# ywq/psnerf

Measured on AMD Instinct MI355X. Metric: ray-samples/sec (train step) on BEAR stage2, higher is better.
Workload: dtype f32

## Files before the change

### include/psnerf_hip.h

```cpp
#ifndef PSNERF_HIP_H
#define PSNERF_HIP_H

#include <stdint.h>

#ifdef __cplusplus
extern "C" {
#endif

#define PSN_OK 0
#define PSN_E_ARG (-1)
#define PSN_E_LAUNCH (-2)
#define PSN_E_UNSUPPORTED (-3)

const char* psn_last_error(void);
int psn_version(void);

int psn_composite_fwd(const float* alpha, const float* rgb, int64_t n_rays, int n_samples, int white_bg,
                      float* weights, float* rgb_out, float* acc_out, void* stream);
int psn_composite_bwd(const float* alpha, const float* rgb, const float* d_rgb_out, const float* d_acc_out,
                      int64_t n_rays, int n_samples, int white_bg, float* d_alpha, float* d_rgb, void* stream);

int psn_pe_encode(const float* x, int64_t n, int n_freqs, float scale, float* out, int out_stride, void* stream);
int psn_app_input(const float* p, const float* v, const float* normal, int64_t n, int n_freqs, float* out, void* stream);

// ... 222 lines not shown
int psn_stage1_rays(const float* pix, const float* camera_mat, int k_ld, const float* world_mat, float radius2, int64_t n,
                    float* cam, float* rays, float* far, void* stream);
int psn_surface_points(const float* d_pred, const int* flags, const float* cam, const float* rays, int64_t n, float* d_i,
                       float* dists, unsigned char* obj_mask, float* points, void* stream);
int psn_stage1_targets(const float* pix, int64_t n, int h, int w, const float* img, const float* mask, const float* mask_valid,
                       const float* normal, const float* norm_mask, const float* world_mat, int use_angle, float cos_thresh,
                       float* rgb_gt, float* mask_gt, unsigned char* mask_valid_out, float* normal_gt,
                       unsigned char* norm_mask_out, void* stream);
#define PSN_COPY2D_MAX 24
typedef struct {
    const float* src; int64_t ld_src;
    float* dst; int64_t ld_dst;
    int rows, cols;
} PsnCopy2dItem;
int psn_copy2d_group(int n_items, const PsnCopy2dItem* items, void* stream);
#define PSN_COPY_BYTES_MAX 24
typedef struct { const void* src; void* dst; int64_t n_bytes; int aligned; } PsnCopyBytesItem;
int psn_copy_bytes_group(int n_items, const PsnCopyBytesItem* items, void* stream);
int psn_mask_count(const unsigned char* mask_a, const unsigned char* mask_b, int64_t n, float* out, void* stream);
int psn_surface_index(const unsigned char* mask, int64_t n, int64_t cap, int64_t* idx, float* count, void* stream);
int psn_inverse_index(const int64_t* idx, int64_t ns, int64_t n_pix, int* inv, const float* count, void* stream);
typedef struct {
    const void* images; int image_type; const float* lut;
    const unsigned char* object_mask; const unsigned char* surface_mask;
    const float* points; const float* normal; const float* visibility; const float* vis_plus; const float* light_direction;
    int64_t hw; int width;
    const int64_t* lidx; int n_lights;
    const int64_t* pix; int64_t pix0; int64_t n;
    const int64_t* vidx; int n_vis;
    float* rgb; unsigned char* object_mask_out; unsigned char* surface_mask_out; float* uv; float* points_out; float* normal_out;
// ... 170 lines not shown
```

### psnerf_amd/csrc/small.hip

```cpp
#include "common.h"

namespace psn {

__device__ __forceinline__ void normalize3(const float x0, const float x1, const float x2, float eps, float& y0, float& y1, float& y2) {
    const float nrm = sqrtf(x0 * x0 + x1 * x1 + x2 * x2);
    const float d = nrm < eps ? eps : nrm;
    y0 = x0 / d; y1 = x1 / d; y2 = x2 / d;
}
__device__ __forceinline__ void normalize3_bwd(const float x0, const float x1, const float x2, const float g0, const float g1,
                                               const float g2, float eps, float& d0, float& d1, float& d2) {
    const float nrm = sqrtf(x0 * x0 + x1 * x1 + x2 * x2);
    const float d = nrm < eps ? eps : nrm;
    d0 = g0 / d; d1 = g1 / d; d2 = g2 / d;
    if (nrm >= eps && nrm > 0.0f) {
        const float s = -((g0 * x0 / d) / d + (g1 * x1 / d) / d + (g2 * x2 / d) / d);
        d0 += x0 / nrm * s; d1 += x1 / nrm * s; d2 += x2 / nrm * s;
    }
}

__global__ __launch_bounds__(256) void normalize_rows_fwd_kernel(const float* __restrict__ x, int64_t n, float eps, float* __restrict__ y) {
    const int64_t i = (int64_t)blockIdx.x * 256 + threadIdx.x;
    if (i >= n) return;
    float y0, y1, y2;
    normalize3(x[3 * i], x[3 * i + 1], x[3 * i + 2], eps, y0, y1, y2);
// ... 224 lines not shown
    Copy2dArgs a;
    a.n = n_items;
    a.start[0] = 0;
    for (int i = 0; i < n_items; ++i) {
        const PsnCopy2dItem& it = items[i];
        PSN_CHECK_ARG(it.src && it.dst && it.rows >= 1 && it.cols >= 1 && it.ld_src >= it.cols && it.ld_dst >= it.cols, "copy2d_group: item %d", i);
        a.it[i] = it;
        a.start[i + 1] = a.start[i] + ((int64_t)it.rows * it.cols + 255) / 256;
    }
    hipLaunchKernelGGL(copy2d_group_kernel, dim3((unsigned)a.start[n_items]), dim3(256), 0, (hipStream_t)stream, a);
    PSN_CHECK_LAUNCH("copy2d_group");
    return PSN_OK;
}

namespace psn {
struct CopyBytesArgs { PsnCopyBytesItem it[PSN_COPY_BYTES_MAX]; int64_t start[PSN_COPY_BYTES_MAX + 1]; int n; };
__global__ __launch_bounds__(256) void copy_bytes_group_kernel(CopyBytesArgs a) {
    int i = 0;
    while (i + 1 < a.n && (int64_t)blockIdx.x >= a.start[i + 1]) ++i;
    const PsnCopyBytesItem it = a.it[i];
    const int64_t b = (int64_t)blockIdx.x - a.start[i];
    const int64_t off = (b * 256 + threadIdx.x) * 16;
    if (off >= it.n_bytes) return;
    const char* s = reinterpret_cast<const char*>(it.src) + off;
    char* d = reinterpret_cast<char*>(it.dst) + off;
    if (it.aligned && off + 16 <= it.n_bytes) {
        *reinterpret_cast<uint4*>(d) = *reinterpret_cast<const uint4*>(s);
    } else {
        const int m = (int)(it.n_bytes - off < 16 ? it.n_bytes - off : 16);
        for (int k = 0; k < m; ++k) d[k] = s[k];
// ... 240 lines not shown
```

### psnerf_amd/fused.py

```python
import math

import torch

from . import hip


class PackCache(object):

    def __init__(self):
        self.epoch = 0
        self._slots = {}

    def key(self, params):
        return (self.epoch,) + tuple((int(p._version), p.data_ptr()) for p in params)

    def invalidate(self):
        self.epoch += 1

    def get(self, slot, params, build, extra=()):
        key = (self.key(params), extra)
        hit = self._slots.get(slot)
        if hit is None or hit[0] != key:
            with torch.no_grad():
                pack = build(hit[1] if hit is not None else None)
# ... 5 lines not shown

    def __init__(self, *args, **kwargs):
        super().__init__(*args, **kwargs)
        self.packs = PackCache()

    def invalidate_packs(self):
        self.packs.invalidate()

    def _apply(self, fn, *a, **k):
        self.packs.invalidate()
        return super()._apply(fn, *a, **k)

    def _load_from_state_dict(self, *a, **k):
        self.packs.invalidate()
        return super()._load_from_state_dict(*a, **k)


def interleave(weights, biases):
    return [t for pair in zip(weights, biases) for t in pair]


class PackedMLP(object):
    def __init__(self, desc, w, b, init_wa=None, init_wb=None, init_bias=None):
        self.desc, self.w, self.b = desc, w, b
        self.init_wa, self.init_wb, self.init_bias = init_wa, init_wb, init_bias
        self.macs_per_row = None

    def on_points(self, points, pe_octaves, pe_scale, out=None, n_rows_dev=None, out_rows=None):
        return hip.mlp_infer_pe(self.desc, self.w, self.b, points, pe_octaves, pe_scale, out=out, macs_per_row=self.macs_per_row,
                                n_rows_dev=n_rows_dev, out_rows=out_rows)
# ... 48 lines not shown

class Transposed(object):

    def __init__(self, w):
        self.w = w.detach()


def _src(w):
    if isinstance(w, Transposed):
        m = w.w
        return m, True, m.shape[1], m.shape[0]
    m = w.detach()
    return m, False, m.shape[0], m.shape[1]


def pack_layers(layers, in_kt_a, in_kt_b, n_out, out_act, device, has_final=True, width=256, reuse=None, x3=False):
    assert width in (64, 128, 256) and (not x3 or width == 256)
    hid = width // 32
    kin = in_kt_a + in_kt_b
    desc = hip.PsnMlpDesc()
    desc.n_layers = len(layers)
    desc.n_out, desc.out_act, desc.in_kt_a, desc.in_kt_b = n_out, out_act, in_kt_a, in_kt_b
    desc.w_format = hip.W_BF16X2 if x3 else hip.W_F32
    assert len(layers) <= hip.MAX_LAYERS
    plan, biases = [], []
    init_wa, init_wb, init_bias = [], [], []
    direct_init_off = None
    off = b_off = 0
    for li, L in enumerate(layers):
        last = has_final and li == len(layers) - 1
        n_mt = (2 if n_out > 32 else 1) if last else hid
# ... 39 lines not shown
        b_buf = _zeros(n_bias, device)
    elif old_b is not None and old_b.numel() == n_bias and old_b.device == w_buf.device and getattr(reuse, 'b_zero', None) == is_zero:
        b_buf, o = old_b, 0
        for bv, z in zip(biases, is_zero):
            if not z:
                side.append((bv, b_buf[o:o + bv.shape[0]]))
            o += bv.shape[0]
    else:
        b_buf = torch.cat(biases).contiguous()
    group = []
    for w, n_mt, k_tiles, o in plan:
        m, tr, r, c = _src(w)
        assert r <= n_mt * 32 and c <= k_tiles * 32, 'pack_layers: block %dx%d does not fit %dx%d' % (r, c, n_mt * 32, k_tiles * 32)
        group.append((m if m.dtype == torch.float32 else m.float(), tr, n_mt, k_tiles, w_buf[o:o + n_mt * k_tiles * 1024],
                      hip.W_BF16X2 if (x3 and n_mt >= 2) else hip.W_F32))
    hip.mlp_pack_layers(group)
    desc.init_stride = width * len(init_wa) if direct_init_off is None else width
    if init_wa:
        def stack(blocks, cols, old):
            shape = (len(blocks) * width, cols)
            buf = old if (old is not None and tuple(old.shape) == shape and old.device == w_buf.device) else torch.zeros(shape, device=device)
            for i, blk in enumerate(blocks):
                assert blk.shape[0] <= width and blk.shape[1] <= cols
                side.append((blk if blk.dtype == torch.float32 else blk.float(), buf[i * width:i * width + blk.shape[0], :blk.shape[1]]))
            return buf
        n_ib = sum(v.shape[0] for v in init_bias)
        old_ib = getattr(reuse, 'init_bias', None)
        if old_ib is not None and old_ib.numel() == n_ib and old_ib.device == w_buf.device:
            ib, o = old_ib, 0
            for v in init_bias:
                side.append((v, ib[o:o + v.shape[0]]))
# ... 4 lines not shown
                       stack(init_wb, in_kt_b * 32, getattr(reuse, 'init_wb', None)) if init_wb else None, ib)
    else:
        pk = PackedMLP(desc, w_buf, b_buf)
    pk.b_zero = is_zero
    if side:
        side = [(a_.detach().contiguous() if a_.dim() == 1 else a_.detach(), d_) for a_, d_ in side]
        if all(a_.is_cuda for a_, _ in side):
            hip.copy2d_group(side)
        else:
            for a_, d_ in side:
                d_.copy_(a_)
    pk.macs_per_row = sum(_src(w)[2] * _src(w)[3] for w, _, _, _ in plan)
    return pk


def pack_relu_mlp(weights, biases, din_a, din_b, skip_at, out_act=hip.OUT_NONE, precompute=True, width=256, reuse=None, x3=False):
    ka = (din_a + 31) // 32
    kb = (din_b + 31) // 32 if din_b > 0 else 0

    def split_in(w):
        if kb == 0:
            return w[:, :din_a]
        wa = _pad_cols(w[:, :din_a], ka * 32)
        return torch.cat([wa, _pad_cols(w[:, din_a:din_a + din_b], kb * 32)], dim=1)

    def in_block(W):
        if precompute:
            return dict(init_a=W[:, :din_a], init_b=W[:, din_a:din_a + din_b] if kb else None)
        return dict(w_in=split_in(W))

    layers = []
    n = len(weights)
    for li in range(n):
        W, b = weights[li].detach(), biases[li].detach()
        act = hip.ACT_RELU if li < n - 1 else hip.ACT_NONE
        if li == 0:
            layers.append(dict(w_act=None, bias=b, act=act, **in_block(W)))
        elif li - 1 == skip_at:
            layers.append(dict(w_act=W[:, :width], bias=b, act=act, **in_block(W[:, width:])))
        else:
            layers.append(dict(w_act=W, bias=b, act=act))
    assert all(L['bias'].shape[0] == width for L in layers[:-1]), 'fused path: every hidden layer must have the given width'
    return pack_layers(layers, ka, kb, weights[-1].shape[0], out_act, weights[0].device, width=width, reuse=reuse, x3=x3)


class PackedBf16(object):

    def __init__(self, desc, w, final_bias):
        self.desc, self.w, self.final_bias = desc, w, final_bias

    def __call__(self, tab_a, n_rows, a_div=1, a_mod=None, tab_b=None, b_div=1, b_mod=1, out=None):
        if a_mod is None:
            a_mod = tab_a.shape[0]
        return hip.mlp_infer_bf16(self.desc, self.w, self.final_bias, tab_a, a_div, a_mod, tab_b, b_div, b_mod, n_rows, out=out)


def pack_relu_mlp_bf16(weights, biases, din_a, din_b, skip_at, out_act=hip.OUT_NONE):
    n = len(weights)
# ... 126 lines not shown
                W, b = -W, -b
        if li == 0:
            layers.append(dict(w_in=W, w_act=None, bias=b, act=act))
        elif li in skips:
            d_x = W.shape[1] - d_pe
            layers.append(dict(w_in=W[:, d_x:] * inv, w_act=W[:, :d_x] * inv, bias=b, act=act))
        else:
            layers.append(dict(w_in=None, w_act=W, bias=b, act=act))
    return pack_layers(layers, ka, 0, 1, out_act, weights[0].device, x3=x3)


def pack_geo_logit(weights, biases, skips, d_pe):
    return pack_geo_occupancy(weights, biases, skips, d_pe, out_act=hip.OUT_NONE, negate=True)


def pack_relu_bwd(weights, skip_at, width=256, bits=False, x3=False):
    n = len(weights)
    dev = weights[0].device
    zeros = _zeros(width, dev)
    act = hip.ACT_RELU_BITS if bits else hip.ACT_RELU_MASK
    layers = [dict(init_a=DIRECT_INIT, init_b=None, w_act=None, bias=zeros, act=act)]
    for l in range(n - 2, 0, -1):
        layers.append(dict(w_act=Transposed(weights[l][:, :width]), bias=zeros, act=act))
    return pack_layers(layers, 1, 0, 0, hip.OUT_NONE, dev, has_final=False, width=width, x3=x3 and width == 256)


def _t(w):
    return Transposed(w)


def pack_geo_chains(weights, biases, skips, d_pe, x3=False):
    n = len(weights)
    assert len(skips) == 1 and weights[1].shape[1] == 256 and weights[n - 1].shape[0] == 257
    sk = skips[0]
    dev = weights[0].device
    W = [w.detach() for w in weights]
    b = [x.detach() for x in biases]
    zeros = _zeros(256, dev)
    ka = (d_pe + 31) // 32
# ... 160 lines not shown
```

### psnerf_amd/hip.py

```python
import ctypes
import os

import torch

from . import cabi

_HERE = os.path.dirname(os.path.abspath(__file__))
LIB_PATH = os.path.join(_HERE, 'libpsnerf_hip.so')

if not os.path.exists(LIB_PATH):
    raise ImportError(
        'psnerf_amd: %s is missing. Build it with `python -m psnerf_amd.build` (hipcc, gfx950). '
        'There is no fallback path.' % LIB_PATH)
_lib = ctypes.CDLL(LIB_PATH)

HEADER_PATH = os.path.join(_HERE, '..', 'include', 'psnerf_hip.h')
if not os.path.exists(HEADER_PATH):
    raise ImportError('psnerf_amd: %s is missing: the binding is derived from it. There is no fallback path.' % HEADER_PATH)

_constants, _structs, SIGNATURES = cabi.parse(HEADER_PATH)
globals().update({_k[len('PSN_'):]: _v for _k, _v in _constants.items()})
globals().update(_structs)
MAX_LAYERS = MLP_MAX_LAYERS
for _name, (_res, _args) in SIGNATURES.items():
# ... 411 lines not shown
    _check(_lib.psn_row_adam(len(items), ctypes.addressof(arr), idx.data_ptr(), idx.numel(), _stream()), 'row_adam')


def normalize_rows_fwd(x, eps=1e-12):
    assert x.dim() == 2 and x.shape[1] == 3 and x.is_contiguous()
    y = torch.empty_like(x)
    _check(_lib.psn_normalize_rows_fwd(_tptr(x, 'x'), x.shape[0], float(eps), y.data_ptr(), _stream()), 'normalize_rows_fwd')
    return y


def normalize_rows_bwd(x, g, eps=1e-12):
    assert x.shape == g.shape and x.shape[1] == 3 and x.is_contiguous() and g.is_contiguous()
    dx = torch.empty_like(x)
    _check(_lib.psn_normalize_rows_bwd(_tptr(x, 'x'), _tptr(g, 'g'), x.shape[0], float(eps), dx.data_ptr(), _stream()), 'normalize_rows_bwd')
    return dx


def light_rows_fwd(dir_table, int_table, idx, eps=1e-12):
    L = idx.shape[0]
    assert dir_table.dim() == 2 and dir_table.shape[1] == 3 and dir_table.is_contiguous() and idx.dtype == torch.int64 and idx.is_contiguous()
    d = torch.empty(L, 3, device=dir_table.device, dtype=torch.float32)
    it = None
    if int_table is not None:
        assert int_table.shape == (dir_table.shape[0], 1) and int_table.is_contiguous()
        it = torch.empty(L, 1, device=dir_table.device, dtype=torch.float32)
    _check(_lib.psn_light_rows_fwd(_tptr(dir_table, 'dir_table'), _tptr(int_table, 'int_table', allow_none=True), _tptr(idx, 'idx', torch.int64), L, float(eps),
                                   d.data_ptr(), None if it is None else it.data_ptr(), _stream()), 'light_rows_fwd')
    return d, it


# ... 1131 lines not shown
```

### psnerf_amd/ops.py

```python
import collections

import torch

from . import fused, hip


HITS = collections.Counter()


def _hit(name):
    HITS[name] += 1


import os as _os0
STRICT = _os0.environ.get('PSN_STRICT', '0') == '1'
FALLBACKS = collections.Counter()


def fallback(name, tensor=None, why=''):
    if tensor is not None and not getattr(tensor, 'is_cuda', False):
        return
    FALLBACKS[name] += 1
    if STRICT:
        raise RuntimeError('psnerf_amd.ops.STRICT: %s left the fused engines on a device tensor%s' % (name, (' (' + why + ')') if why else ''))
# ... 208 lines not shown
class SplitRows(torch.autograd.Function):

    @staticmethod
    def forward(ctx, t, k):
        ctx.k, ctx.shape = k, t.shape
        return t[:k], t[k:]

    @staticmethod
    def backward(ctx, ga, gb):
        k, shape = ctx.k, ctx.shape
        if ga is None:
            ga = gb.new_zeros((k,) + tuple(shape[1:]))
        if gb is None:
            gb = ga.new_zeros((shape[0] - k,) + tuple(shape[1:]))
        return torch.cat([ga, gb], dim=0), None


class ScatterRows(torch.autograd.Function):

    @staticmethod
    def forward(ctx, idx, inv, specs, *rows):
        _hit('ScatterRows')
        ctx.set_materialize_grads(False)
        ctx.specs, ctx.n_pix, ctx.ns = specs, inv.numel(), idx.numel()
        ctx.save_for_backward(idx, inv)
        return tuple(hip.scatter_rows(list(specs), [r.detach() for r in rows], inv, inv.numel(), idx.numel()))

    @staticmethod
    def backward(ctx, *grads):
        idx, inv = ctx.saved_tensors
# ... 285 lines not shown
def mf_shade(light_dir, view, normal, albedo, rough, light_int, vis, f0):
    return MFShade.apply(light_dir, view, normal, albedo, rough, light_int, vis, f0)


RELU_SIGN_BITS = True


def _sign_bits(rows, n, device):
    return [torch.empty(rows, 4, device=device, dtype=torch.int64) for _ in range(n)]


class VisibilityPair(torch.autograd.Function):

    @staticmethod
    def launch(pe_x, pe_l, n_shade, in_cols, skip_at, params, need_grad, packed=None, live_count=None):
        Ws, bs = params[0::2], params[1::2]
        Ns, LV = pe_x.shape[0], pe_l.shape[0]
        V = LV - n_shade
        n = len(Ws)
        din_half = in_cols.numel() // 2
        with torch.no_grad():
            if packed is None:
                packed = fused.pack_relu_mlp(list(Ws), list(bs), din_half, din_half, skip_at)
            save = [torch.empty(V * Ns, 256, device=pe_x.device) for _ in range(n - 1)] if (need_grad and V > 0) else None
            bits = _sign_bits(V * Ns, n - 1, pe_x.device) if (save is not None and RELU_SIGN_BITS) else None
            out = packed(pe_x, LV * Ns, a_div=1, a_mod=Ns, tab_b=pe_l, b_div=Ns, b_mod=LV, save=save, save_row0=n_shade * Ns,
                         live=None if (live_count is None or Ns % 64 != 0) else (live_count, Ns),
                         save_bits=bits)
        return out, (save, bits) if save is not None else None

    @staticmethod
    def forward(ctx, pe_x, pe_l, n_shade, in_cols, skip_at, pre, *params):
        _hit('VisibilityPair')
        Ns, LV = pe_x.shape[0], pe_l.shape[0]
        V = LV - n_shade
        n = len(params) // 2
        need = any(ctx.needs_input_grad[6:])
        out, dumps = pre if pre is not None else VisibilityPair.launch(pe_x, pe_l, n_shade, in_cols, skip_at, params, need)
        save, bits = dumps if (need and dumps is not None) else (None, None)
        if save is not None:
            ctx.save_for_backward(pe_x, pe_l[n_shade:], in_cols, *save, *params)
        ctx.bits = bits
        ctx.n, ctx.skip_at, ctx.V, ctx.saved = n, skip_at, V, save is not None
        ctx.contiguous_cols = bool(getattr(in_cols, '_psn_contiguous_pair', False))
        vis, vis_t = out[:n_shade * Ns], out[n_shade * Ns:]
        ctx.mark_non_differentiable(vis)
        return vis, vis_t

    @staticmethod
    def backward(ctx, _g_vis, g):
        n, V = ctx.n, ctx.V
        if not ctx.saved or g is None:
            return (None,) * (6 + 2 * n)
        sv = ctx.saved_tensors
        pe_x, pe_lv, in_cols = sv[0], sv[1], sv[2]
        H = sv[3:3 + n - 1]
        Ws = sv[3 + n - 1::2]
        Ns = pe_x.shape[0]
        Q = V * Ns
        half = in_cols.numel() // 2
        cols_a, cols_b = in_cols[:half], in_cols[half:] - pe_x.shape[1]
        contiguous_cols = ctx.contiguous_cols
        grads = [None] * (2 * n)
        g = g.contiguous()

        bits = ctx.bits
        chain = fused.pack_relu_bwd(list(Ws), ctx.skip_at, bits=bits is not None, x3=CHAIN_X3)
        DZ = [torch.empty(Q, 256, device=g.device) for _ in range(n - 1)]
        chain(None, Q, a_div=1, a_mod=Q, rank_init=(g.reshape(Q, 1), Ws[n - 1].reshape(1, -1).contiguous()),
              mask=[(bits if bits is not None else H)[n - 2 - j] for j in range(n - 1)], save=DZ, save_row0=0)
        grads[2 * (n - 1)] = hip.colsum(H[n - 2], row_weight=g)
        grads[2 * (n - 1) + 1] = _rowsum_small(g)
        items = []
        where = []
        xl = {}
        for li in range(n - 2, -1, -1):
            dz = DZ[n - 2 - li]
            if li > 0:
                items.append(dict(A=dz, B=H[li - 1], colsum=True))
                where.append((li, 'w'))
            if li == 0 or li - 1 == ctx.skip_at:
                if V <= 16:
# ... 182 lines not shown
        d_feat = torch.empty(Q, 256, device=dev)
        d_normal = chains['bwd'](None, Q, a_div=1, a_mod=Q, rank_init=(g, Ws[n - 1].contiguous()),
                                 mask=[H[n - 2 - j] for j in range(n - 1)] + [None, None], save=DZ + [d_feat])
        dz0 = DZ[n - 2]
        items = [dict(A=dz0, B=x[:, :d_x], colsum=True), dict(A=dz0, B=feat)]
        items += [dict(A=DZ[n - 2 - l], B=H[l - 1], colsum=True) for l in range(1, n - 1)]
        res = hip.gemm_tn_grouped(items)
        grads = [torch.cat([res[0][0], res[1][0]], dim=1), res[0][1]]
        for l in range(1, n - 1):
            grads += [res[l + 1][0], res[l + 1][1]]
        grads += [hip.colsum(H[n - 2], row_weight=g), _rowsum_small(g)]
        return (None, d_normal, d_feat, None, None) + tuple(grads)


class FusedReluNet(torch.autograd.Function):

    @staticmethod
    def pack(Ws, bs, din, skip_at, final_sigmoid, width):
        with torch.no_grad():
            return fused.pack_relu_mlp(list(Ws), list(bs), din, 0, skip_at,
                                       out_act=hip.OUT_SIGMOID if final_sigmoid else hip.OUT_NONE, precompute=False, width=width)

    @staticmethod
    def forward(ctx, pe, din, skip_at, final_sigmoid, width, packed, *params):
        _hit('FusedReluNet')
        Ws, bs = params[0::2], params[1::2]
        n = len(Ws)
        Q = pe.shape[0]
        if packed is None:
            packed = FusedReluNet.pack(Ws, bs, din, skip_at, final_sigmoid, width)
        need = any(ctx.needs_input_grad[6:])
        H = [torch.empty(Q, width, device=pe.device) for _ in range(n - 1)] if need else None
        bits = _sign_bits(Q, n - 1, pe.device) if (need and RELU_SIGN_BITS) else None
        out = packed(pe, Q, save=H, save_bits=bits)
        if need:
            ctx.save_for_backward(pe, out, *H, *Ws)
            ctx.meta = (n, din, skip_at, final_sigmoid, width)
            ctx.bits = bits
        return out

    @staticmethod
    def backward(ctx, g):
        n, din, skip_at, final_sigmoid, width = ctx.meta
        sv = ctx.saved_tensors
        pe, out = sv[0], sv[1]
        H = sv[2:2 + n - 1]
        Ws = sv[2 + n - 1:]
        Q, dev = pe.shape[0], pe.device
        g = g.contiguous()
        if final_sigmoid:
            g = torch.ops.aten.sigmoid_backward(g, out)
        bits = ctx.bits
        chain = fused.pack_relu_bwd(list(Ws), skip_at, width=width, bits=bits is not None, x3=CHAIN_X3)
        DZ = [torch.empty(Q, width, device=dev) for _ in range(n - 1)]
        masks = [(bits if bits is not None else H)[n - 2 - j] for j in range(n - 1)]
        if Ws[n - 1].shape[0] <= 4:
            chain(None, Q, a_div=1, a_mod=Q, rank_init=(g, Ws[n - 1].contiguous()), mask=masks, save=DZ)
        else:
            dh = hip.gemm(g, Ws[n - 1].contiguous())
            chain(None, Q, a_div=1, a_mod=Q, init_a_direct=dh, mask=masks, save=DZ)
        x_in = pe[:, :din]
        items = [dict(A=g, B=H[n - 2], colsum=True)]
        where = [(n - 1, 'w')]
        for l in range(n - 2, -1, -1):
            dz = DZ[n - 2 - l]
            if l == 0:
                items.append(dict(A=dz, B=x_in, colsum=True))
                where.append((0, 'w'))
# ... 156 lines not shown
```

### psnerf_amd/stage2/renderer.py

```python
import contextlib
import os

import numpy as np
import torch
import torch.nn as nn
import torch.nn.functional as F

from .. import fused, hip, ops

PE_STRIDE = 64


def camera_rays(uv, pose, intrinsics):
    fx, fy = intrinsics[:, 0, 0], intrinsics[:, 1, 1]
    cx, cy = intrinsics[:, 0, 2], intrinsics[:, 1, 2]
    z = torch.ones_like(uv[:, :, 0])
    x = (uv[:, :, 0] - cx.unsqueeze(-1)) / fx.unsqueeze(-1) * z
    y = (uv[:, :, 1] - cy.unsqueeze(-1)) / fy.unsqueeze(-1) * z
    R = pose[:, :3, :3]
    d = x.unsqueeze(-1) * R[:, None, :, 0] + y.unsqueeze(-1) * R[:, None, :, 1] + z.unsqueeze(-1) * R[:, None, :, 2]
    return F.normalize(d, dim=2), pose[:, :3, 3]


class MLP(fused.PackCached, nn.Module):
# ... 18 lines not shown

    FUSED = True

    def _fused_shape(self):
        Ws = [l.weight for l in self.linears]
        return (self.FUSED and self.width in (64, 128, 256) and self.din <= 64 and Ws[-1].shape[0] <= 32
                and all(w.shape[0] == self.width for w in Ws[:-1]))

    def _fusable(self, x_padded, in_cols):
        return (self._fused_shape() and x_padded.shape[1] == 64 and not x_padded.requires_grad
                and in_cols.numel() == self.din and len(self.linears) <= 11)

    def prepack(self):
        if not (self._fused_shape() and self.linears[0].weight.is_cuda):
            return None
        return self.packs.get('fwd', self.parameters(), lambda _: ops.FusedReluNet.pack(
            *self.weights(), self.din, self._skip_index(), self.final == 'sigmoid', self.width))

    def forward(self, x_padded, in_cols):
        Ws, bs = self.weights()
        if self._fusable(x_padded, in_cols):
            return ops.FusedReluNet.apply(x_padded, self.din, self._skip_index(), self.final == 'sigmoid', self.width,
                                          self.prepack(), *fused.interleave(Ws, bs))
        if self.FUSED:
            ops.fallback('stage2.MLP -> layer-wise GEMMs', x_padded, 'width %d, %d layers, input %s' % (self.width, len(Ws), tuple(x_padded.shape)))
        return ops.relu_mlp(x_padded, in_cols, self._skip_index(), self.final == 'sigmoid', Ws, bs)


class SGBasis(nn.Module):

    def __init__(self, nbasis=9, specular_rgb=False):
        super().__init__()
        self.nbasis, self.specular_rgb = nbasis, specular_rgb
        self.lobe = nn.Parameter(torch.tensor([np.exp(i) for i in range(2, 11)], dtype=torch.float32),
                                 requires_grad=False)


# ... 99 lines not shown
            return self._visibility_rows_lowp(mode, pe_x, pe_l)
        if fused_ok and net.width == 256:
            return ops.FusedPairMLP.apply(pe_x, pe_l, cols, net._skip_index(), *fused.interleave(Ws, bs))
        if fused_ok:
            ops.fallback('stage2.visibility rows -> expanded [L Ns, 128] input', pe_x, 'visibility_net width %d' % net.width)
        ns, nl = pe_x.shape[0], pe_l.shape[0]
        x = torch.cat([pe_x.tile(nl, 1), pe_l.repeat_interleave(ns, dim=0)], dim=1)
        return net(x, cols)

    def _visibility_pair_args(self, pe_x, light_dir, light_vis_train):
        pe_l = self._pe(torch.cat([light_dir.detach(), light_vis_train.detach()], dim=0), self.n_freqs)
        net = self.visibility_net
        cols = self._cols(self.n_freqs, pe_x.device, pair=True)
        return pe_x.detach(), pe_l, light_dir.shape[0], cols, net._skip_index(), fused.interleave(*net.weights())

    def _visibility_prepack(self):
        net = self.visibility_net
        if net.width != 256 or not net.linears[0].weight.is_cuda:
            return None
        return self._vis_pack('fp32', lambda prev, *net_args: fused.pack_relu_mlp(*net_args, reuse=prev))

    def _vis_pack(self, slot, build):
        net = self.visibility_net

        def make(prev):
            Ws, bs = net.weights()
            half = 3 + 6 * self.n_freqs
            return build(prev, list(Ws), list(bs), half, half, net._skip_index())
        return self.packs.get(slot, net.parameters(), make)

    def _vis_out_act(self):
        return hip.OUT_SIGMOID if self.visibility_net.final == 'sigmoid' else hip.OUT_NONE

    @torch.no_grad()
    def _visibility_rows_bf16(self, pe_x, pe_l):
# ... 17 lines not shown
        return rows[mode](pe_x, pe_l)

    def _memo(self, tag, input, fn):
        cache = self._eval_cache
        if cache is None or torch.is_grad_enabled():
            return fn()
        key = (tag,) + tuple((input[k].data_ptr(), input[k]._version) for k in ('points', 'surface_mask', 'uv')) \
            + self.packs.key(self.parameters())
        if key not in cache:
            cache[key] = fn()
        return cache[key]

    def _visibility_pair_launch(self, pe_x, light_dir, light_vis_train, live_count=None):
        a = self._visibility_pair_args(pe_x, light_dir, light_vis_train)
        need = any(p.requires_grad for p in a[5])
        return a, ops.VisibilityPair.launch(a[0], a[1], a[2], a[3], a[4], [p.detach() for p in a[5]], need,
                                            packed=self._visibility_prepack(), live_count=live_count)

    def _visibility_pair(self, pe_x, light_dir, light_vis_train, launched=None):
        if launched is not None:
            a, pre = launched
        else:
            a, pre = self._visibility_pair_args(pe_x, light_dir, light_vis_train), None
        return ops.VisibilityPair.apply(a[0], a[1], a[2], a[3], a[4], pre, *a[5])

    def forward(self, input, albedo_new=None, basis_new=None, noise=None):
        noise = noise or {}
        uv, pose, intr = input['uv'], input['pose'], input['intrinsics']
        object_mask = input['object_mask']
        device = uv.device
        surface_mask, points, normals = input['surface_mask'], input['points'], input['normal']
        idx = input.get('surface_idx')
# ... 29 lines not shown
            if pair_ok:
                pe_x = self._pe(surf, self.n_freqs)
                if self.overlap_small_nets and surf.is_cuda:
                    side = self._side.get(device)
                    if side is None:
                        side = self._side[device] = torch.cuda.Stream(device=device)
                    side.wait_stream(torch.cuda.current_stream(device))
                mode = 'bf16x3' if self.train_vis_bf16x3 else 'bf16x6' if self.train_vis_bf16x6 else 'bf16' if self.train_vis_bf16 else None
                if mode is not None:
                    pe_l0 = self._pe(ld0.detach(), self.n_freqs)
                    vis_bf16 = self._visibility_rows_lowp(mode, pe_x, pe_l0)
                    vis_pair = self._visibility_pair_launch(pe_x, ld0[:0], lv0)
                else:
                    vis_pair = self._visibility_pair_launch(pe_x, ld0, lv0, live_count=input.get('surface_count'))
        on_side = (lambda: torch.cuda.stream(side)) if side is not None else contextlib.nullcontext
        if self.normal_mlp:
            normal_pred = ones3()
            if ns > 0:
              with on_side():
                cols_n = self._cols(self.n_freqs_n, device)
                pe_n = (lambda: pe_x) if (pe_x is not None and self.n_freqs_n == self.n_freqs) else (lambda: self._pe(surf, self.n_freqs_n))
                if self.normal_jitter_std > 0 and torch.is_grad_enabled():
                    nz = noise.get('normal')
                    if nz is None:
                        nz = torch.empty_like(surf).normal_(0.0, self.normal_jitter_std)
                    pe_both_n = torch.cat([pe_n(), self._pe(surf + nz, self.n_freqs_n)], dim=0)
                    normal_s, nj = ops.SplitRows.apply(ops.normalize_rows(self.normal_net(pe_both_n, cols_n)), ns)
                    normal_pred = scatter(normal_pred, normal_s)
                    out_n['normal_jitter'] = scatter(ones3(), nj)
                else:
                    normal_s = self._memo('normal', input, lambda: ops.normalize_rows(self.normal_net(pe_n(), cols_n)))
                    normal_pred = scatter(normal_pred, normal_s)
                    if self.normal_jitter_std > 0:
                        nz = noise.get('normal')
                        if nz is None:
                            nz = torch.empty_like(surf).normal_(0.0, self.normal_jitter_std)
                        nj = self._memo('normal_jitter', input, lambda: ops.normalize_rows(
                            self.normal_net(self._pe(surf + nz, self.n_freqs_n), cols_n)))
                        out_n['normal_jitter'] = scatter(ones3(), nj)
            out_n['normal_pred'] = normal_pred

        sg = self.render_model == 'sgbasis'
        lnum = input['light_direction'].shape[0]
        rgb_values = ones3(lnum)
        albedo_values = ones3()
        rough_values = ones3(lnum) if sg else ones3()
        weight_values = _Dense(0.0, 1, self.nbasis) if sg else None
        vis_values = ones3(lnum)
        jitter = None
        vis_t_pre = None
        if ns > 0:
            normal = gather(normals) if not self.normal_mlp else normal_s
            with on_side():
                if (uv.is_cuda and uv.shape[0] == 1 and uv.dtype == torch.float32 and tuple(pose.shape[1:]) == (4, 4)
                        and tuple(intr.shape[1:]) == (4, 4)):
                    pts2c = hip.camera_rays(uv.contiguous(), pose.contiguous().float(), intr.contiguous().float(), idx, scale=-1.0)
                else:
                    ray_dirs, _ = camera_rays(uv, pose, intr)
                    pts2c = -gather(ray_dirs)
            light_dir = input['light_direction']
            cols = self._cols(self.n_freqs, device)
            if pe_x is None:
                pe_x = self._memo('pe_x', input, lambda: self._pe(surf, self.n_freqs))
            pe_j = None
            with on_side():
              if self.xyz_jitter_std > 0:
                nz = noise.get('xyz')
                if nz is None:
                    nz = torch.empty_like(surf).normal_(0.0, self.xyz_jitter_std)
                def brdf_both():
                    pe_both = torch.cat([pe_x, self._pe(surf + nz, self.n_freqs)], dim=0)
                    return self.albedo_net(pe_both, cols), self.rough_net(pe_both, cols)
                albedo_both, rough_both = self._memo('brdf_both', input, brdf_both)
                albedo, albedo_j = ops.SplitRows.apply(albedo_both, ns)
                if sg:
                    rough_both = F.relu(rough_both)
                rough, rough_j = ops.SplitRows.apply(rough_both, ns)
              else:
                albedo, rough = self._memo('brdf', input, lambda: (self.albedo_net(pe_x, cols), self.rough_net(pe_x, cols)))
              if albedo_new is not None:
                albedo = torch.from_numpy(albedo_new).to(device)[None].expand_as(albedo)
              if sg:
                weights = rough if self.xyz_jitter_std > 0 else F.relu(rough)
                if basis_new is not None:
                    wn = torch.zeros_like(weights)
                    if self.specular_rgb:
                        wn.view(-1, 3, self.nbasis // 3)[:, :, basis_new] = 2 ** basis_new / 100
                    else:
                        wn.view(-1, 1, self.nbasis)[:, :, basis_new] = 2 ** basis_new / 100
                    weights = wn.reshape(-1, self.nbasis)
                weight_values = scatter(weight_values, weights)
            if side is not None:
                main = torch.cuda.current_stream(device)
                main.wait_stream(side)
                for t_ in (pts2c, normal_s, albedo_both if self.xyz_jitter_std > 0 else albedo, rough_both if self.xyz_jitter_std > 0 else rough,
                           weights if sg else None, out_n.get('normal_jitter').rows if 'normal_jitter' in out_n else None):
                    if torch.is_tensor(t_):
                        t_.record_stream(main)
            light_int = input.get('light_intensity', self.light_int)
            vis = None
            vis_for_rgb = None
            vis_t_pre = None
            if self.visibility:
                detach = self.conf.get_bool('train.vis_rgb_detach', default=False)
                if pair_ok:
                    if vis_bf16 is not None:
                        _none, vis_t_pre = self._visibility_pair(pe_x, light_dir[:0], lv0, launched=vis_pair)
                        vis = vis_bf16
                    else:
                        vis, vis_t_pre = self._visibility_pair(pe_x, light_dir, lv0, launched=vis_pair)
                else:
                    vis = self._visibility_rows(pe_x, light_dir, fused_ok=True)
                vis_for_rgb = vis.detach() if detach else vis
            if sg:
                rgb, spec = ops.sg_shade(light_dir, pts2c, normal, albedo, weights, self.sgbasis.lobe, light_int,
                                         vis_for_rgb, self.specular_rgb)
            else:
                rgb = ops.mf_shade(light_dir, pts2c, normal, albedo, rough, light_int, vis_for_rgb, self.f0)
            rgb_values = scatter(rgb_values, rgb)
            if vis is not None:
                vis_values = scatter(vis_values, vis.expand(rgb.shape))
            albedo_values = scatter(albedo_values, albedo)
            if sg:
                rough_values = scatter(rough_values, spec.expand(-1, 3))
            else:
                rough_values = scatter(rough_values, rough.expand(-1, 3))
            if self.xyz_jitter_std > 0:
                aj = scatter(ones3(), albedo_j)
                if sg:
                    rj = scatter(_Dense(1.0, 1, self.nbasis), rough_j)
                    r_ori = weight_values
                else:
                    rj = scatter(ones3(), rough_j.expand(-1, 3))
                    r_ori = rough_values
                jitter = {'albedo_values': albedo_values, 'albedo_jitter': aj,
                          'rough_values': r_ori, 'rough_jitter': rj}

        out = {
            'points': points, 'object_mask': object_mask, 'network_object_mask': surface_mask,
            'sg_rgb_values': rgb_values, 'normal_values': normals,
            'sg_diffuse_albedo_values': albedo_values, 'sg_specular_rgb_values': rough_values,
# ... 52 lines not shown
```

Before: 112.9 million.

## Fuse head split/activation backward into one kernel and cache backward chain packs

Adds a grouped head_bwd HIP kernel and a HeadSplit autograd function. Together they replace the SplitRows, ReLU and sigmoid_backward ops on the albedo, rough and normal heads with one launch that sums the gradient branches and applies the activation derivative. Separately, the backward weight-chain packs for the BRDF MLPs and the visibility MLP are now built alongside the forward packs and cached, instead of being repacked on every backward pass. This cuts per-step kernel launches and repacking work, at the cost of more complex autograd plumbing and cache-key handling.

```diff
diff --git a/include/psnerf_hip.h b/include/psnerf_hip.h
--- a/include/psnerf_hip.h
+++ b/include/psnerf_hip.h
@@ -260,6 +260,18 @@
     int rows, cols;
 } PsnCopy2dItem;
 int psn_copy2d_group(int n_items, const PsnCopy2dItem* items, void* stream);
+#define PSN_HEAD_MAX 4
+#define PSN_HEAD_NONE 0
+#define PSN_HEAD_RELU 1
+#define PSN_HEAD_SIGMOID 2
+typedef struct {
+    const float* g_a; const float* g_b; const float* g_j;
+    const float* out;
+    float* dst;
+    int64_t ns, nj;
+    int cols, mode;
+} PsnHeadItem;
+int psn_head_bwd(int n_items, const PsnHeadItem* items, void* stream);
 #define PSN_COPY_BYTES_MAX 24
 typedef struct { const void* src; void* dst; int64_t n_bytes; int aligned; } PsnCopyBytesItem;
 int psn_copy_bytes_group(int n_items, const PsnCopyBytesItem* items, void* stream);
diff --git a/psnerf_amd/csrc/small.hip b/psnerf_amd/csrc/small.hip
--- a/psnerf_amd/csrc/small.hip
+++ b/psnerf_amd/csrc/small.hip
@@ -262,6 +262,54 @@
 }
 
 namespace psn {
+struct HeadArgs { PsnHeadItem it[PSN_HEAD_MAX]; int64_t start[PSN_HEAD_MAX + 1]; int n; };
+__global__ __launch_bounds__(256) void head_bwd_kernel(HeadArgs a) {
+    int i = 0;
+    while (i + 1 < a.n && (int64_t)blockIdx.x >= a.start[i + 1]) ++i;
+    const PsnHeadItem it = a.it[i];
+    const int64_t e = ((int64_t)blockIdx.x - a.start[i]) * 256 + threadIdx.x;
+    const int64_t n_base = it.ns * it.cols;
+    if (e >= n_base + it.nj * it.cols) return;
+    float g = 0.0f;
+    if (e < n_base) {
+        if (it.g_a != nullptr && it.g_b != nullptr) g = it.g_a[e] + it.g_b[e];
+        else if (it.g_a != nullptr) g = it.g_a[e];
+        else if (it.g_b != nullptr) g = it.g_b[e];
+    } else if (it.g_j != nullptr) {
+        g = it.g_j[e - n_base];
+    }
+    if (it.mode == PSN_HEAD_RELU) {
+        g = it.out[e] <= 0.0f ? 0.0f : g;
+    } else if (it.mode == PSN_HEAD_SIGMOID) {
+        const float o = it.out[e];
+        g = __fmul_rn(__fmul_rn(g, __fsub_rn(1.0f, o)), o);
+    }
+    it.dst[e] = g;
+}
+}
+
+extern "C" int psn_head_bwd(int n_items, const PsnHeadItem* items, void* stream) {
+    using namespace psn;
+    PSN_CHECK_ARG(items && n_items >= 1 && n_items <= PSN_HEAD_MAX, "head_bwd: n_items=%d", n_items);
+    HeadArgs a;
+    a.n = n_items;
+    a.start[0] = 0;
+    for (int i = 0; i < n_items; ++i) {
+        const PsnHeadItem& it = items[i];
+        PSN_CHECK_ARG(it.dst && it.ns >= 0 && it.nj >= 0 && it.cols >= 1, "head_bwd: item %d: bad shape or null destination", i);
+        PSN_CHECK_ARG(it.mode == PSN_HEAD_NONE || ((it.mode == PSN_HEAD_RELU || it.mode == PSN_HEAD_SIGMOID) && it.out), "head_bwd: item %d: mode %d%s", i,
+                      it.mode, it.out ? "" : " needs the forward output");
+        a.it[i] = it;
+        a.start[i + 1] = a.start[i] + ((it.ns + it.nj) * it.cols + 255) / 256;
+    }
+    PSN_CHECK_ARG(a.start[n_items] < (1ll << 31), "head_bwd: too many elements");
+    if (a.start[n_items] == 0) return PSN_OK;
+    hipLaunchKernelGGL(head_bwd_kernel, dim3((unsigned)a.start[n_items]), dim3(256), 0, (hipStream_t)stream, a);
+    PSN_CHECK_LAUNCH("head_bwd");
+    return PSN_OK;
+}
+
+namespace psn {
 struct CopyBytesArgs { PsnCopyBytesItem it[PSN_COPY_BYTES_MAX]; int64_t start[PSN_COPY_BYTES_MAX + 1]; int n; };
 __global__ __launch_bounds__(256) void copy_bytes_group_kernel(CopyBytesArgs a) {
     int i = 0;
diff --git a/psnerf_amd/fused.py b/psnerf_amd/fused.py
--- a/psnerf_amd/fused.py
+++ b/psnerf_amd/fused.py
@@ -43,6 +43,35 @@
     def _load_from_state_dict(self, *a, **k):
         self.packs.invalidate()
         return super()._load_from_state_dict(*a, **k)
+
+
+class TrainPacks(object):
+
+    def __init__(self, fwd, chain, chain_key):
+        self.fwd, self.chain, self.chain_key = fwd, chain, chain_key
+
+    def chain_for(self, bits, x3):
+        return self.chain if self.chain_key == (bool(bits), bool(x3)) else None
+
+
+def pack_with_chain(cache, params, slot, build_fwd, chain_slot, build_chain, chain_key):
+    params = list(params)
+
+    def both(prev):
+        plan = []
+        fwd = build_fwd(prev, plan)
+        cache.get(chain_slot, params, lambda _prev: build_chain(plan), extra=chain_key)
+        if plan:
+            hip.mlp_pack_layers(plan)
+        return fwd
+    fwd = cache.get(slot, params, both)
+
+    def alone(_prev):
+        plan = []
+        chain = build_chain(plan)
+        hip.mlp_pack_layers(plan)
+        return chain
+    return TrainPacks(fwd, cache.get(chain_slot, params, alone, extra=chain_key), chain_key)
 
 
 def interleave(weights, biases):
@@ -121,7 +150,7 @@
     return m, False, m.shape[0], m.shape[1]
 
 
-def pack_layers(layers, in_kt_a, in_kt_b, n_out, out_act, device, has_final=True, width=256, reuse=None, x3=False):
+def pack_layers(layers, in_kt_a, in_kt_b, n_out, out_act, device, has_final=True, width=256, reuse=None, x3=False, defer=None):
     assert width in (64, 128, 256) and (not x3 or width == 256)
     hid = width // 32
     kin = in_kt_a + in_kt_b
@@ -191,7 +220,10 @@
         assert r <= n_mt * 32 and c <= k_tiles * 32, 'pack_layers: block %dx%d does not fit %dx%d' % (r, c, n_mt * 32, k_tiles * 32)
         group.append((m if m.dtype == torch.float32 else m.float(), tr, n_mt, k_tiles, w_buf[o:o + n_mt * k_tiles * 1024],
                       hip.W_BF16X2 if (x3 and n_mt >= 2) else hip.W_F32))
-    hip.mlp_pack_layers(group)
+    if defer is not None:
+        defer.extend(group)
+    else:
+        hip.mlp_pack_layers(group)
     desc.init_stride = width * len(init_wa) if direct_init_off is None else width
     if init_wa:
         def stack(blocks, cols, old):
@@ -226,7 +258,7 @@
     return pk
 
 
-def pack_relu_mlp(weights, biases, din_a, din_b, skip_at, out_act=hip.OUT_NONE, precompute=True, width=256, reuse=None, x3=False):
+def pack_relu_mlp(weights, biases, din_a, din_b, skip_at, out_act=hip.OUT_NONE, precompute=True, width=256, reuse=None, x3=False, defer=None):
     ka = (din_a + 31) // 32
     kb = (din_b + 31) // 32 if din_b > 0 else 0
 
@@ -253,7 +285,7 @@
         else:
             layers.append(dict(w_act=W, bias=b, act=act))
     assert all(L['bias'].shape[0] == width for L in layers[:-1]), 'fused path: every hidden layer must have the given width'
-    return pack_layers(layers, ka, kb, weights[-1].shape[0], out_act, weights[0].device, width=width, reuse=reuse, x3=x3)
+    return pack_layers(layers, ka, kb, weights[-1].shape[0], out_act, weights[0].device, width=width, reuse=reuse, x3=x3, defer=defer)
 
 
 class PackedBf16(object):
@@ -410,7 +442,7 @@
     return pack_geo_occupancy(weights, biases, skips, d_pe, out_act=hip.OUT_NONE, negate=True)
 
 
-def pack_relu_bwd(weights, skip_at, width=256, bits=False, x3=False):
+def pack_relu_bwd(weights, skip_at, width=256, bits=False, x3=False, defer=None):
     n = len(weights)
     dev = weights[0].device
     zeros = _zeros(width, dev)
@@ -418,7 +450,7 @@
     layers = [dict(init_a=DIRECT_INIT, init_b=None, w_act=None, bias=zeros, act=act)]
     for l in range(n - 2, 0, -1):
         layers.append(dict(w_act=Transposed(weights[l][:, :width]), bias=zeros, act=act))
-    return pack_layers(layers, 1, 0, 0, hip.OUT_NONE, dev, has_final=False, width=width, x3=x3 and width == 256)
+    return pack_layers(layers, 1, 0, 0, hip.OUT_NONE, dev, has_final=False, width=width, x3=x3 and width == 256, defer=defer)
 
 
 def _t(w):
diff --git a/psnerf_amd/hip.py b/psnerf_amd/hip.py
--- a/psnerf_amd/hip.py
+++ b/psnerf_amd/hip.py
@@ -449,6 +449,23 @@
     dx = torch.empty_like(x)
     _check(_lib.psn_normalize_rows_bwd(_tptr(x, 'x'), _tptr(g, 'g'), x.shape[0], float(eps), dx.data_ptr(), _stream()), 'normalize_rows_bwd')
     return dx
+
+
+def head_bwd(items):
+    assert 1 <= len(items) <= HEAD_MAX
+    arr = (PsnHeadItem * len(items))()
+    res = []
+    for k, (e, (g_a, g_b, g_j, out, ns, nj, cols, mode)) in enumerate(zip(arr, items)):
+        for t, rows in ((g_a, ns), (g_b, ns), (g_j, nj), (out, ns + nj)):
+            assert t is None or tuple(t.shape) == (rows, cols), 'head_bwd: item %d: %s is not [%d, %d]' % (k, tuple(t.shape), rows, cols)
+        dev = next(t for t in (g_a, g_b, g_j, out) if t is not None).device
+        dst = torch.empty(ns + nj, cols, device=dev, dtype=torch.float32)
+        e.g_a, e.g_b, e.g_j = (_tptr(t, 'head_bwd: gradient', allow_none=True) for t in (g_a, g_b, g_j))
+        e.out = _tptr(out, 'head_bwd: out', allow_none=mode == HEAD_NONE)
+        e.dst, e.ns, e.nj, e.cols, e.mode = dst.data_ptr(), ns, nj, cols, mode
+        res.append(dst)
+    _check(_lib.psn_head_bwd(len(items), ctypes.addressof(arr), _stream()), 'head_bwd')
+    return res
 
 
 def light_rows_fwd(dir_table, int_table, idx, eps=1e-12):
diff --git a/psnerf_amd/ops.py b/psnerf_amd/ops.py
--- a/psnerf_amd/ops.py
+++ b/psnerf_amd/ops.py
@@ -246,6 +246,39 @@
         if gb is None:
             gb = ga.new_zeros((shape[0] - k,) + tuple(shape[1:]))
         return torch.cat([ga, gb], dim=0), None
+
+
+class HeadSplit(torch.autograd.Function):
+
+    @staticmethod
+    def forward(ctx, ns, modes, *outs):
+        _hit('HeadSplit')
+        assert len(modes) == len(outs) and all(t.dim() == 2 and t.shape[0] >= ns for t in outs)
+        ctx.set_materialize_grads(False)
+        acts = [torch.relu(t) if m == hip.HEAD_RELU else t for t, m in zip(outs, modes)]
+        ctx.ns, ctx.modes, ctx.shapes = ns, tuple(modes), [tuple(t.shape) for t in outs]
+        ctx.save_for_backward(*[a for a, m in zip(acts, modes) if m != hip.HEAD_NONE])
+        res = []
+        for a in acts:
+            res += [a[:ns], a[:ns], a[ns:]]
+        return tuple(res)
+
+    @staticmethod
+    def backward(ctx, *grads):
+        saved = iter(ctx.saved_tensors)
+        items, where = [], []
+        for k, (mode, shape) in enumerate(zip(ctx.modes, ctx.shapes)):
+            out = next(saved) if mode != hip.HEAD_NONE else None
+            g = [None if t is None else t.contiguous() for t in grads[3 * k:3 * k + 3]]
+            if not ctx.needs_input_grad[2 + k] or all(t is None for t in g):
+                continue
+            items.append((g[0], g[1], g[2], out, ctx.ns, shape[0] - ctx.ns, shape[1], mode))
+            where.append(k)
+        res = [None] * len(ctx.modes)
+        if items:
+            for k, d in zip(where, hip.head_bwd(items)):
+                res[k] = d
+        return (None, None) + tuple(res)
 
 
 class ScatterRows(torch.autograd.Function):
@@ -561,6 +594,8 @@
 
     @staticmethod
     def launch(pe_x, pe_l, n_shade, in_cols, skip_at, params, need_grad, packed=None, live_count=None):
+        if isinstance(packed, fused.TrainPacks):
+            packed = packed.fwd
         Ws, bs = params[0::2], params[1::2]
         Ns, LV = pe_x.shape[0], pe_l.shape[0]
         V = LV - n_shade
@@ -583,7 +618,8 @@
         V = LV - n_shade
         n = len(params) // 2
         need = any(ctx.needs_input_grad[6:])
-        out, dumps = pre if pre is not None else VisibilityPair.launch(pe_x, pe_l, n_shade, in_cols, skip_at, params, need)
+        out, dumps = pre[:2] if pre is not None else VisibilityPair.launch(pe_x, pe_l, n_shade, in_cols, skip_at, params, need)
+        ctx.packs = pre[2] if (pre is not None and len(pre) > 2) else None
         save, bits = dumps if (need and dumps is not None) else (None, None)
         if save is not None:
             ctx.save_for_backward(pe_x, pe_l[n_shade:], in_cols, *save, *params)
@@ -612,7 +648,9 @@
         g = g.contiguous()
 
         bits = ctx.bits
-        chain = fused.pack_relu_bwd(list(Ws), ctx.skip_at, bits=bits is not None, x3=CHAIN_X3)
+        chain = ctx.packs.chain_for(bits is not None, CHAIN_X3) if ctx.packs is not None else None
+        if chain is None:
+            chain = fused.pack_relu_bwd(list(Ws), ctx.skip_at, bits=bits is not None, x3=CHAIN_X3)
         DZ = [torch.empty(Q, 256, device=g.device) for _ in range(n - 1)]
         chain(None, Q, a_div=1, a_mod=Q, rank_init=(g.reshape(Q, 1), Ws[n - 1].reshape(1, -1).contiguous()),
               mask=[(bits if bits is not None else H)[n - 2 - j] for j in range(n - 1)], save=DZ, save_row0=0)
@@ -825,12 +863,17 @@
 
 
 class FusedReluNet(torch.autograd.Function):
-
-    @staticmethod
-    def pack(Ws, bs, din, skip_at, final_sigmoid, width):
+    SIGMOID_BWD_DONE = 2
+
+    @staticmethod
+    def pack(Ws, bs, din, skip_at, final_sigmoid, width, defer=None):
         with torch.no_grad():
             return fused.pack_relu_mlp(list(Ws), list(bs), din, 0, skip_at,
-                                       out_act=hip.OUT_SIGMOID if final_sigmoid else hip.OUT_NONE, precompute=False, width=width)
+                                       out_act=hip.OUT_SIGMOID if final_sigmoid else hip.OUT_NONE, precompute=False, width=width, defer=defer)
+
+    @staticmethod
+    def chain_key():
+        return (bool(RELU_SIGN_BITS), bool(CHAIN_X3))
 
     @staticmethod
     def forward(ctx, pe, din, skip_at, final_sigmoid, width, packed, *params):
@@ -838,6 +881,9 @@
         Ws, bs = params[0::2], params[1::2]
         n = len(Ws)
         Q = pe.shape[0]
+        train_packs = packed if isinstance(packed, fused.TrainPacks) else None
+        if train_packs is not None:
+            packed = train_packs.fwd
         if packed is None:
             packed = FusedReluNet.pack(Ws, bs, din, skip_at, final_sigmoid, width)
         need = any(ctx.needs_input_grad[6:])
@@ -848,6 +894,7 @@
             ctx.save_for_backward(pe, out, *H, *Ws)
             ctx.meta = (n, din, skip_at, final_sigmoid, width)
             ctx.bits = bits
+            ctx.packs = train_packs
         return out
 
     @staticmethod
@@ -859,10 +906,12 @@
         Ws = sv[2 + n - 1:]
         Q, dev = pe.shape[0], pe.device
         g = g.contiguous()
-        if final_sigmoid:
+        if final_sigmoid and final_sigmoid != FusedReluNet.SIGMOID_BWD_DONE:
             g = torch.ops.aten.sigmoid_backward(g, out)
         bits = ctx.bits
-        chain = fused.pack_relu_bwd(list(Ws), skip_at, width=width, bits=bits is not None, x3=CHAIN_X3)
+        chain = ctx.packs.chain_for(bits is not None, CHAIN_X3) if ctx.packs is not None else None
+        if chain is None:
+            chain = fused.pack_relu_bwd(list(Ws), skip_at, width=width, bits=bits is not None, x3=CHAIN_X3)
         DZ = [torch.empty(Q, width, device=dev) for _ in range(n - 1)]
         masks = [(bits if bits is not None else H)[n - 2 - j] for j in range(n - 1)]
         if Ws[n - 1].shape[0] <= 4:
diff --git a/psnerf_amd/stage2/renderer.py b/psnerf_amd/stage2/renderer.py
--- a/psnerf_amd/stage2/renderer.py
+++ b/psnerf_amd/stage2/renderer.py
@@ -56,13 +56,25 @@
     def prepack(self):
         if not (self._fused_shape() and self.linears[0].weight.is_cuda):
             return None
-        return self.packs.get('fwd', self.parameters(), lambda _: ops.FusedReluNet.pack(
-            *self.weights(), self.din, self._skip_index(), self.final == 'sigmoid', self.width))
-
-    def forward(self, x_padded, in_cols):
+
+        def fwd(_prev, defer=None):
+            return ops.FusedReluNet.pack(*self.weights(), self.din, self._skip_index(), self.final == 'sigmoid', self.width, defer=defer)
+        if not (torch.is_grad_enabled() and any(p.requires_grad for p in self.parameters())):
+            return self.packs.get('fwd', self.parameters(), fwd)
+        bits, x3 = key = ops.FusedReluNet.chain_key()
+        return fused.pack_with_chain(self.packs, self.parameters(), 'fwd', fwd, 'bwd', lambda defer: fused.pack_relu_bwd(
+            self.weights()[0], self._skip_index(), width=self.width, bits=bits, x3=x3, defer=defer), key)
+
+    def head_mode(self, x_padded, in_cols):
+        return hip.HEAD_SIGMOID if (self.final == 'sigmoid' and self._fusable(x_padded, in_cols)) else hip.HEAD_NONE
+
+    def forward(self, x_padded, in_cols, sigmoid_bwd_done=False):
         Ws, bs = self.weights()
         if self._fusable(x_padded, in_cols):
-            return ops.FusedReluNet.apply(x_padded, self.din, self._skip_index(), self.final == 'sigmoid', self.width,
+            final = self.final == 'sigmoid'
+            if final and sigmoid_bwd_done:
+                final = ops.FusedReluNet.SIGMOID_BWD_DONE
+            return ops.FusedReluNet.apply(x_padded, self.din, self._skip_index(), final, self.width,
                                           self.prepack(), *fused.interleave(Ws, bs))
         if self.FUSED:
             ops.fallback('stage2.MLP -> layer-wise GEMMs', x_padded, 'width %d, %d layers, input %s' % (self.width, len(Ws), tuple(x_padded.shape)))
@@ -192,11 +204,18 @@
         cols = self._cols(self.n_freqs, pe_x.device, pair=True)
         return pe_x.detach(), pe_l, light_dir.shape[0], cols, net._skip_index(), fused.interleave(*net.weights())
 
-    def _visibility_prepack(self):
+    def _visibility_prepack(self, train=False):
         net = self.visibility_net
         if net.width != 256 or not net.linears[0].weight.is_cuda:
             return None
-        return self._vis_pack('fp32', lambda prev, *net_args: fused.pack_relu_mlp(*net_args, reuse=prev))
+        if not train:
+            return self._vis_pack('fp32', lambda prev, *net_args: fused.pack_relu_mlp(*net_args, reuse=prev))
+        half = 3 + 6 * self.n_freqs
+        bits, x3 = key = ops.FusedReluNet.chain_key()
+        return fused.pack_with_chain(
+            self.packs, net.parameters(), 'fp32',
+            lambda prev, defer: fused.pack_relu_mlp(*net.weights(), half, half, net._skip_index(), reuse=prev, defer=defer),
+            'fp32_bwd', lambda defer: fused.pack_relu_bwd(net.weights()[0], net._skip_index(), bits=bits, x3=x3, defer=defer), key)
 
     def _vis_pack(self, slot, build):
         net = self.visibility_net
@@ -244,8 +263,10 @@
     def _visibility_pair_launch(self, pe_x, light_dir, light_vis_train, live_count=None):
         a = self._visibility_pair_args(pe_x, light_dir, light_vis_train)
         need = any(p.requires_grad for p in a[5])
-        return a, ops.VisibilityPair.launch(a[0], a[1], a[2], a[3], a[4], [p.detach() for p in a[5]], need,
-                                            packed=self._visibility_prepack(), live_count=live_count)
+        packs = self._visibility_prepack(train=need and torch.is_grad_enabled())
+        out, dumps = ops.VisibilityPair.launch(a[0], a[1], a[2], a[3], a[4], [p.detach() for p in a[5]], need,
+                                               packed=packs, live_count=live_count)
+        return a, (out, dumps, packs if isinstance(packs, fused.TrainPacks) else None)
 
     def _visibility_pair(self, pe_x, light_dir, light_vis_train, launched=None):
         if launched is not None:
@@ -305,20 +326,31 @@
                 else:
                     vis_pair = self._visibility_pair_launch(pe_x, ld0, lv0, live_count=input.get('surface_count'))
         on_side = (lambda: torch.cuda.stream(side)) if side is not None else contextlib.nullcontext
+        normal_both = None
+        normal_d = None
         if self.normal_mlp:
             normal_pred = ones3()
             if ns > 0:
               with on_side():
                 cols_n = self._cols(self.n_freqs_n, device)
                 pe_n = (lambda: pe_x) if (pe_x is not None and self.n_freqs_n == self.n_freqs) else (lambda: self._pe(surf, self.n_freqs_n))
-                if self.normal_jitter_std > 0 and torch.is_grad_enabled():
-                    nz = noise.get('normal')
-                    if nz is None:
-                        nz = torch.empty_like(surf).normal_(0.0, self.normal_jitter_std)
-                    pe_both_n = torch.cat([pe_n(), self._pe(surf + nz, self.n_freqs_n)], dim=0)
-                    normal_s, nj = ops.SplitRows.apply(ops.normalize_rows(self.normal_net(pe_both_n, cols_n)), ns)
-                    normal_pred = scatter(normal_pred, normal_s)
-                    out_n['normal_jitter'] = scatter(ones3(), nj)
+                jit_n = self.normal_jitter_std > 0
+                if torch.is_grad_enabled() and (jit_n or any(p.requires_grad for p in self.normal_net.parameters())):
+                    pe_in_n = pe_n()
+                    if jit_n:
+                        nz = noise.get('normal')
+                        if nz is None:
+                            nz = torch.empty_like(surf).normal_(0.0, self.normal_jitter_std)
+                        pe_in_n = torch.cat([pe_in_n, self._pe(surf + nz, self.n_freqs_n)], dim=0)
+                    normal_both = ops.normalize_rows(self.normal_net(pe_in_n, cols_n))
+                    if not (self.xyz_jitter_std > 0):
+                        normal_s, normal_d, nj = ops.HeadSplit.apply(ns, (hip.HEAD_NONE,), normal_both)
+                        normal_both = None
+                        normal_pred = scatter(normal_pred, normal_d)
+                        if jit_n:
+                            out_n['normal_jitter'] = scatter(ones3(), nj)
+                    elif jit_n:
+                        out_n['normal_jitter'] = None
                 else:
                     normal_s = self._memo('normal', input, lambda: ops.normalize_rows(self.normal_net(pe_n(), cols_n)))
                     normal_pred = scatter(normal_pred, normal_s)
@@ -341,7 +373,6 @@
         jitter = None
         vis_t_pre = None
         if ns > 0:
-            normal = gather(normals) if not self.normal_mlp else normal_s
             with on_side():
                 if (uv.is_cuda and uv.shape[0] == 1 and uv.dtype == torch.float32 and tuple(pose.shape[1:]) == (4, 4)
                         and tuple(intr.shape[1:]) == (4, 4)):
@@ -361,31 +392,38 @@
                     nz = torch.empty_like(surf).normal_(0.0, self.xyz_jitter_std)
                 def brdf_both():
                     pe_both = torch.cat([pe_x, self._pe(surf + nz, self.n_freqs)], dim=0)
-                    return self.albedo_net(pe_both, cols), self.rough_net(pe_both, cols)
-                albedo_both, rough_both = self._memo('brdf_both', input, brdf_both)
-                albedo, albedo_j = ops.SplitRows.apply(albedo_both, ns)
-                if sg:
-                    rough_both = F.relu(rough_both)
-                rough, rough_j = ops.SplitRows.apply(rough_both, ns)
+                    modes = (self.albedo_net.head_mode(pe_both, cols), hip.HEAD_RELU if sg else self.rough_net.head_mode(pe_both, cols))
+                    return (self.albedo_net(pe_both, cols, sigmoid_bwd_done=True), self.rough_net(pe_both, cols, sigmoid_bwd_done=True), modes)
+                albedo_both, rough_both, modes = self._memo('brdf_both', input, brdf_both)
+                heads = ops.HeadSplit.apply(ns, modes + ((hip.HEAD_NONE,) if normal_both is not None else ()),
+                                            albedo_both, rough_both, *([normal_both] if normal_both is not None else []))
+                albedo, albedo_d, albedo_j, rough, rough_d, rough_j = heads[:6]
+                if normal_both is not None:
+                    normal_s, normal_d, nj = heads[6:]
+                    if 'normal_jitter' in out_n:
+                        out_n['normal_jitter'] = scatter(ones3(), nj)
+                    out_n['normal_pred'] = scatter(out_n['normal_pred'], normal_d)
               else:
                 albedo, rough = self._memo('brdf', input, lambda: (self.albedo_net(pe_x, cols), self.rough_net(pe_x, cols)))
+                albedo_d, rough_d = albedo, rough
               if albedo_new is not None:
-                albedo = torch.from_numpy(albedo_new).to(device)[None].expand_as(albedo)
+                albedo = albedo_d = torch.from_numpy(albedo_new).to(device)[None].expand_as(albedo)
               if sg:
-                weights = rough if self.xyz_jitter_std > 0 else F.relu(rough)
+                weights, weights_d = (rough, rough_d) if self.xyz_jitter_std > 0 else (F.relu(rough),) * 2
                 if basis_new is not None:
                     wn = torch.zeros_like(weights)
                     if self.specular_rgb:
                         wn.view(-1, 3, self.nbasis // 3)[:, :, basis_new] = 2 ** basis_new / 100
                     else:
                         wn.view(-1, 1, self.nbasis)[:, :, basis_new] = 2 ** basis_new / 100
-                    weights = wn.reshape(-1, self.nbasis)
-                weight_values = scatter(weight_values, weights)
+                    weights = weights_d = wn.reshape(-1, self.nbasis)
+                weight_values = scatter(weight_values, weights_d)
+            normal = gather(normals) if not self.normal_mlp else normal_s
             if side is not None:
                 main = torch.cuda.current_stream(device)
                 main.wait_stream(side)
-                for t_ in (pts2c, normal_s, albedo_both if self.xyz_jitter_std > 0 else albedo, rough_both if self.xyz_jitter_std > 0 else rough,
-                           weights if sg else None, out_n.get('normal_jitter').rows if 'normal_jitter' in out_n else None):
+                for t_ in (pts2c, normal_s, albedo, rough, weights if sg else None,
+                           out_n['normal_jitter'].rows if out_n.get('normal_jitter') is not None else None):
                     if torch.is_tensor(t_):
                         t_.record_stream(main)
             light_int = input.get('light_intensity', self.light_int)
@@ -411,11 +449,11 @@
             rgb_values = scatter(rgb_values, rgb)
             if vis is not None:
                 vis_values = scatter(vis_values, vis.expand(rgb.shape))
-            albedo_values = scatter(albedo_values, albedo)
+            albedo_values = scatter(albedo_values, albedo_d)
             if sg:
                 rough_values = scatter(rough_values, spec.expand(-1, 3))
             else:
-                rough_values = scatter(rough_values, rough.expand(-1, 3))
+                rough_values = scatter(rough_values, rough_d.expand(-1, 3))
             if self.xyz_jitter_std > 0:
                 aj = scatter(ones3(), albedo_j)
                 if sg:
```

Measured after the change: 113.4 million, median of 6. Within noise of the previous version (+0.4%).
